# Createroner/InSAR-Unet-CA

Hardware: AMD Instinct MI355X
Metric: InSAR tiles/sec (fwd+bwd) U-Net-CA 256x256 (higher is better)
Workload: dtype bf16; 1 GPU; U-Net-CA (in=2, classes=2, use_se) bf16, batch 16x2x256x256 per GPU, Dice+CE + Adam(lr=1e-4) training on synthetic InSAR tiles; global_batch=16, parallelism=dp1

## Files before the change

insar_unet_ca_amd/csrc/wgrad.hip:

```cpp
#include "common.h"

typedef __attribute__((ext_vector_type(8))) short bf16x8_t;
typedef __attribute__((ext_vector_type(4))) short s16x4_t;
typedef __attribute__((ext_vector_type(4))) float f32x4_t;

#define WG_BKP 64

struct WgradArgs {
  const char* x; const char* dy; const int32_t* tabx; const int32_t* tabdy; float* part;
  long long ksteps;
  int nsplit, ntaps, steps_per_split;
  int Cx, cx_off, Cin; int Cdy, cdy_off, Cout;
  int mtc, ntc;
  int offx[12], offdy[12];
  long long tabx_tap_stride;
};


template <int RB>
__device__ __forceinline__ int wg_swz(int row) {
  if constexpr (RB == 256) return (row & 7) << 1;
  else return ((row >> 1) & 3) << 1;
}

template <typename T, int TM, int TN, int NW>
struct WgradCfg {
  static constexpr int ES = sizeof(T);
  static constexpr int THREADS = NW * 64;
  static constexpr int SUBX = (TM * ES > 256) ? TM * ES / 256 : 1, SUBY = (TN * ES > 256) ? TN * ES / 256 : 1;
  static constexpr int RBX = TM * ES / SUBX, RBY = TN * ES / SUBY;
  static constexpr int X_STAGE = WG_BKP * TM * ES, Y_STAGE = WG_BKP * TN * ES;
  static constexpr int STAGE = X_STAGE + Y_STAGE;
  static constexpr int LDS_BYTES = 2 * STAGE + 128;
  static constexpr int CPRX = RBX / 16, CPRY = RBY / 16;
  static constexpr int NX = X_STAGE / 16 / THREADS;
  static constexpr int NY = Y_STAGE / 16 / THREADS;
  static constexpr int MTW = TM / 32, NTW = TN / (NW / 2) / 16;
};

template <typename T, int TM, int TN, int NW>
__global__ __launch_bounds__(NW * 64, (NW == 4 ? 2 : 1)) void wgrad_kernel(WgradArgs a) {
  using Cfg = WgradCfg<T, TM, TN, NW>;
  constexpr int WG_THREADS = Cfg::THREADS;
  constexpr int ES = Cfg::ES;
  constexpr int MTW = Cfg::MTW, NTW = Cfg::NTW;
  extern __shared__ __attribute__((aligned(16))) char smem[];
  int* soff = (int*)(smem + 2 * Cfg::STAGE);

  const int tid = threadIdx.x, lane = tid & 63, wave = tid >> 6;
  int t;
  {
    const int nwg = gridDim.x, bid = blockIdx.x;
    const int q = nwg >> 3, r = nwg & 7, xcd = bid & 7;
    t = (xcd < r ? xcd * (q + 1) : r * (q + 1) + (xcd - r) * q) + (bid >> 3);
  }
  const int tap = t % a.ntaps; t /= a.ntaps;
  const int ni = t % a.ntc; t /= a.ntc;
  const int mi = t % a.mtc; t /= a.mtc;
  const int split = t;

  if (tid == WG_THREADS - 1) {
#pragma unroll
    for (int i = 0; i < 12; ++i) { soff[i] = a.offx[i]; soff[12 + i] = a.offdy[i]; }
  }
  __syncthreads();
  const long long offx = soff[tap], offdy = soff[12 + tap];

  const long long ks0 = (long long)split * a.steps_per_split;
  long long ks1 = ks0 + a.steps_per_split;
  if (ks1 > a.ksteps) ks1 = a.ksteps;

  const long long xcol = ((long long)a.cx_off + mi * TM) * ES;
  const long long ycol = ((long long)a.cdy_off + ni * TN) * ES;
  int xrow_i[Cfg::NX], yrow_i[Cfg::NY];
  int xoff_i[Cfg::NX], yoff_i[Cfg::NY];
#pragma unroll
  for (int i = 0; i < Cfg::NX; ++i) {
    const int q = i * WG_THREADS + tid;
    const int sub = q / (WG_BKP * Cfg::CPRX), row = (q / Cfg::CPRX) % WG_BKP, pos = q % Cfg::CPRX;
    xrow_i[i] = row;
    xoff_i[i] = sub * Cfg::RBX + (pos ^ wg_swz<Cfg::RBX>(row)) * 16;
  }
#pragma unroll
  for (int i = 0; i < Cfg::NY; ++i) {
    const int q = i * WG_THREADS + tid;
    const int sub = q / (WG_BKP * Cfg::CPRY), row = (q / Cfg::CPRY) % WG_BKP, pos = q % Cfg::CPRY;
    yrow_i[i] = row;
    yoff_i[i] = sub * Cfg::RBY + (pos ^ wg_swz<Cfg::RBY>(row)) * 16;
  }
  const char* xbase = a.x + offx * a.Cx * ES + xcol;
  const char* ybase = a.dy + offdy * a.Cdy * ES + ycol;
  const long long xpitch = (long long)a.Cx * ES, ypitch = (long long)a.Cdy * ES;

  int32_t px[Cfg::NX], py[Cfg::NY];
  const int32_t* tabx_tap = a.tabx + (long long)tap * a.tabx_tap_stride;
  auto load_tabs = [&](long long ks) {
#pragma unroll
    for (int i = 0; i < Cfg::NX; ++i) px[i] = tabx_tap[ks * WG_BKP + xrow_i[i]];
#pragma unroll
    for (int i = 0; i < Cfg::NY; ++i) py[i] = a.tabdy[ks * WG_BKP + yrow_i[i]];
  };
  const uint32_t lds0 = lds_offset_of(smem);
  auto stage = [&](int buf) {
    const uint32_t lx = lds0 + buf * Cfg::STAGE + wave * 1024;
#pragma unroll
    for (int i = 0; i < Cfg::NX; ++i)
      lds_dma16_untracked(xbase + (long long)px[i] * xpitch + xoff_i[i], lx + i * (WG_THREADS * 16));
    const uint32_t ly = lx + Cfg::X_STAGE;
#pragma unroll
    for (int i = 0; i < Cfg::NY; ++i)
      lds_dma16_untracked(ybase + (long long)py[i] * ypitch + yoff_i[i], ly + i * (WG_THREADS * 16));
  };

  f32x4_t acc[MTW][NTW];
#pragma unroll
  for (int i = 0; i < MTW; ++i)
#pragma unroll
    for (int j = 0; j < NTW; ++j) acc[i][j] = (f32x4_t){0.f, 0.f, 0.f, 0.f};

  const int wm = wave & 1, wn = wave >> 1;
  const int r16 = lane & 15, kq = lane >> 4;

  if (ks0 < ks1) {
    load_tabs(ks0);
    stage(0);
    if (ks0 + 1 < ks1) load_tabs(ks0 + 1);
    dma_drain_and_barrier();
    for (long long ks = ks0; ks < ks1; ++ks) {
      const int buf = (int)((ks - ks0) & 1);
      if (ks + 1 < ks1) {
        stage(buf ^ 1);
        if (ks + 2 < ks1) load_tabs(ks + 2);
      }
      const char* sX = smem + buf * Cfg::STAGE;
      const char* sY = sX + Cfg::X_STAGE;
      if constexpr (ES == 2) {
#pragma unroll
        for (int s = 0; s < 2; ++s) {
          bf16x8_t xf[MTW], yf[NTW];
#pragma unroll
          for (int h = 0; h < 2; ++h) {
            const int sel = h ^ (kq & 1);
            const int row = s * 32 + kq * 8 + sel * 4 + (r16 >> 2);
#pragma unroll
            for (int mt = 0; mt < MTW; ++mt) {
              const int colw = (wm * (TM / 2) + mt * 16 + (r16 & 3) * 4) * 2;
              int sub = 0, colb = colw;
              if constexpr (Cfg::SUBX > 1) { sub = colw / Cfg::RBX; colb = colw % Cfg::RBX; }
              const int pc = (colb >> 4) ^ wg_swz<Cfg::RBX>(row);
              const char* p = sX + sub * (WG_BKP * Cfg::RBX) + row * Cfg::RBX + pc * 16 + (colb & 15);
              s16x4_t v = __builtin_amdgcn_ds_read_tr16_b64_v4i16((__attribute__((address_space(3))) s16x4_t*)p);
              xf[mt][4 * h + 0] = v[0]; xf[mt][4 * h + 1] = v[1]; xf[mt][4 * h + 2] = v[2]; xf[mt][4 * h + 3] = v[3];
            }
#pragma unroll
            for (int nt = 0; nt < NTW; ++nt) {
              const int colw = (wn * (NTW * 16) + nt * 16 + (r16 & 3) * 4) * 2;
              int sub = 0, colb = colw;
              if constexpr (Cfg::SUBY > 1) { sub = colw / Cfg::RBY; colb = colw % Cfg::RBY; }
              const int pc = (colb >> 4) ^ wg_swz<Cfg::RBY>(row);
              const char* p = sY + sub * (WG_BKP * Cfg::RBY) + row * Cfg::RBY + pc * 16 + (colb & 15);
              s16x4_t v = __builtin_amdgcn_ds_read_tr16_b64_v4i16((__attribute__((address_space(3))) s16x4_t*)p);
              yf[nt][4 * h + 0] = v[0]; yf[nt][4 * h + 1] = v[1]; yf[nt][4 * h + 2] = v[2]; yf[nt][4 * h + 3] = v[3];
            }
          }
#pragma unroll
          for (int mt = 0; mt < MTW; ++mt)
#pragma unroll
            for (int nt = 0; nt < NTW; ++nt)
              acc[mt][nt] = __builtin_amdgcn_mfma_f32_16x16x32_bf16(xf[mt], yf[nt], acc[mt][nt], 0, 0, 0);
        }
      } else {
#pragma unroll 4
        for (int jj = 0; jj < WG_BKP / 4; ++jj) {
          const int row = jj * 4 + kq;
          float xf[MTW], yf[NTW];
#pragma unroll
          for (int mt = 0; mt < MTW; ++mt) {
            const int colw = (wm * (TM / 2) + mt * 16 + r16) * 4;
            const int sub = colw / Cfg::RBX, colb = colw % Cfg::RBX;
            const int pc = (colb >> 4) ^ wg_swz<Cfg::RBX>(row);
            xf[mt] = *(const float*)(sX + sub * (WG_BKP * Cfg::RBX) + row * Cfg::RBX + pc * 16 + (colb & 15));
          }
#pragma unroll
          for (int nt = 0; nt < NTW; ++nt) {
            const int colw = (wn * (NTW * 16) + nt * 16 + r16) * 4;
            const int sub = colw / Cfg::RBY, colb = colw % Cfg::RBY;
            const int pc = (colb >> 4) ^ wg_swz<Cfg::RBY>(row);
            yf[nt] = *(const float*)(sY + sub * (WG_BKP * Cfg::RBY) + row * Cfg::RBY + pc * 16 + (colb & 15));
          }
#pragma unroll
          for (int mt = 0; mt < MTW; ++mt)
#pragma unroll
            for (int nt = 0; nt < NTW; ++nt)
              acc[mt][nt] = __builtin_amdgcn_mfma_f32_16x16x4f32(xf[mt], yf[nt], acc[mt][nt], 0, 0, 0);
        }
      }
      dma_drain_and_barrier();
    }
  }

  float* out = a.part + ((long long)split * a.ntaps + tap) * a.Cout * a.Cin;
#pragma unroll
  for (int mt = 0; mt < MTW; ++mt)
#pragma unroll
    for (int nt = 0; nt < NTW; ++nt) {
      const int ci = mi * TM + wm * (TM / 2) + mt * 16 + kq * 4;
      const int co = ni * TN + wn * (NTW * 16) + nt * 16 + r16;
      *(f32x4_t*)(out + (long long)co * a.Cin + ci) = acc[mt][nt];
    }
}

template <typename T, int TM, int TN, int NW>
static int launch_wgrad(WgradArgs& a, hipStream_t s) {
  using Cfg = WgradCfg<T, TM, TN, NW>;
  static std::atomic<uint64_t> attr_mask{0};
  {
    hipError_t e = insar_set_lds_once(attr_mask, (const void*)wgrad_kernel<T, TM, TN, NW>, Cfg::LDS_BYTES);
    if (e != hipSuccess) INSAR_FAIL(-(int)e, "insar_wgrad: hipFuncSetAttribute: %s", hipGetErrorString(e));
  }
  a.mtc = a.Cin / TM; a.ntc = a.Cout / TN;
  const long long grid = (long long)a.nsplit * a.ntaps * a.mtc * a.ntc;
  if (grid > 0x7fffffffLL) INSAR_FAIL(INSAR_E_SHAPE, "insar_wgrad: grid too large");
  hipLaunchKernelGGL((wgrad_kernel<T, TM, TN, NW>), dim3((unsigned)grid), dim3(Cfg::THREADS), Cfg::LDS_BYTES, s, a);
  INSAR_CHECK_LAUNCH("insar_wgrad");
  return INSAR_OK;
}

extern "C" int insar_wgrad_tile(int32_t C, int32_t dtype) {
  if (dtype != INSAR_BF16) return (C % 128) == 0 ? 128 : 64;
  const int cap = insar_knob(KNOB_WGRAD_TILE_MAX);
  if (cap > 0 && cap < 256) return (C % 128) == 0 ? 128 : 64;
  return (C % 256) == 0 ? 256 : ((C % 128) == 0 ? 128 : 64);
}

static void wgrad_tile_pair(int Cin, int Cout, int dtype, int& tm, int& tn) {
  tm = insar_wgrad_tile(Cin, dtype); tn = insar_wgrad_tile(Cout, dtype);
  if (dtype != INSAR_BF16) { if (!(tm == 128 && tn == 128)) tm = tn = 64; return; }
  if (tm == 256 && tn == 256) return;
  tm = tm > 128 ? 128 : tm; tn = tn > 128 ? 128 : tn;
}
extern "C" int insar_wgrad_tile_pair(int32_t Cin, int32_t Cout, int32_t dtype) {
  int tm, tn;
  wgrad_tile_pair(Cin, Cout, dtype, tm, tn);
  return (tm << 16) | tn;
}

extern "C" int insar_wgrad(const InsarWgrad* d, void* stream) {
  if (!d || !d->x.ptr || !d->dy.ptr || !d->tabx || !d->tabdy || !d->part) INSAR_FAIL(INSAR_E_ARG, "insar_wgrad: null pointer");
  int rc;
  if ((rc = insar_check_act(&d->x, "insar_wgrad", "x"))) return rc;
  if ((rc = insar_check_act(&d->dy, "insar_wgrad", "dy"))) return rc;
  if (d->x.dtype != d->dy.dtype) INSAR_FAIL(INSAR_E_DTYPE, "insar_wgrad: x/dy dtype differ");
  if (d->Mpad < WG_BKP || d->Mpad % WG_BKP) INSAR_FAIL(INSAR_E_SHAPE, "insar_wgrad: Mpad must be a positive multiple of 64");
  if (d->nsplit < 1 || d->ntaps < 1 || d->ntaps > 12) INSAR_FAIL(INSAR_E_SHAPE, "insar_wgrad: nsplit/ntaps");
  const int Cin = d->x.c_len, Cout = d->dy.c_len;
  if (Cin % 64 || Cout % 64) INSAR_FAIL(INSAR_E_SHAPE, "insar_wgrad: Cin=%d/Cout=%d must be multiples of 64", Cin, Cout);
  WgradArgs a;
  a.x = (const char*)d->x.ptr; a.dy = (const char*)d->dy.ptr; a.tabx = d->tabx; a.tabdy = d->tabdy; a.part = d->part;
  a.ksteps = d->Mpad / WG_BKP;
  a.nsplit = d->nsplit; a.ntaps = d->ntaps;
  a.steps_per_split = (int)((a.ksteps + d->nsplit - 1) / d->nsplit);
  a.Cx = d->x.C; a.cx_off = d->x.c_off; a.Cin = Cin;
  a.Cdy = d->dy.C; a.cdy_off = d->dy.c_off; a.Cout = Cout;
  for (int t = 0; t < 12; ++t) { a.offx[t] = t < d->ntaps ? d->offx[t] : 0; a.offdy[t] = t < d->ntaps ? d->offdy[t] : 0; }
  a.tabx_tap_stride = d->tabx_tap_stride;
  hipStream_t s = (hipStream_t)stream;
  int tm, tn;
  wgrad_tile_pair(Cin, Cout, d->x.dtype, tm, tn);
  if (d->x.dtype == INSAR_BF16) {
    if (tm == 256 && tn == 256) return launch_wgrad<bf16_t, 256, 256, 8>(a, s);
    if (tm == 128 && tn == 128) return launch_wgrad<bf16_t, 128, 128, 4>(a, s);
    if (tm == 128) return launch_wgrad<bf16_t, 128, 64, 4>(a, s);
    if (tn == 128) return launch_wgrad<bf16_t, 64, 128, 4>(a, s);
    return launch_wgrad<bf16_t, 64, 64, 4>(a, s);
  }
  if (tm == 128 && tn == 128) return launch_wgrad<float, 128, 128, 8>(a, s);
  return launch_wgrad<float, 64, 64, 4>(a, s);
}

__global__ void wgrad_fold_kernel(const float4* __restrict__ in, float4* __restrict__ out, long long slab4, int nsplit,
                                  int group) {
  const int g = blockIdx.y;
  const int s0 = g * group;
  int s1 = s0 + group; if (s1 > nsplit) s1 = nsplit;
  for (long long e = blockIdx.x * (long long)blockDim.x + threadIdx.x; e < slab4; e += (long long)gridDim.x * blockDim.x) {
    float4 acc = make_float4(0.f, 0.f, 0.f, 0.f);
#pragma unroll 8
    for (int sp = s0; sp < s1; ++sp) {
      const float4 v = in[(long long)sp * slab4 + e];
      acc.x += v.x; acc.y += v.y; acc.z += v.z; acc.w += v.w;
    }
    out[(long long)g * slab4 + e] = acc;
  }
}

extern "C" int insar_wgrad_fold(const float* part_in, float* part_out, int64_t slab_floats, int32_t nsplit, int32_t group,
                                void* stream) {
  if (!part_in || !part_out) INSAR_FAIL(INSAR_E_ARG, "insar_wgrad_fold: null pointer");
  if (slab_floats < 4 || (slab_floats & 3) || nsplit < 1 || group < 1) INSAR_FAIL(INSAR_E_SHAPE, "insar_wgrad_fold: bad shape");
  const long long slab4 = slab_floats / 4;
  const int groups = (nsplit + group - 1) / group;
  dim3 grid(insar_grid_cap((slab4 + 255) / 256, 1024), groups);
  hipLaunchKernelGGL(wgrad_fold_kernel, grid, dim3(256), 0, (hipStream_t)stream, (const float4*)part_in, (float4*)part_out,
                     slab4, nsplit, group);
  INSAR_CHECK_LAUNCH("insar_wgrad_fold");
  return INSAR_OK;
}

#define WR_CIT 128
template <bool VEC>
__global__ void wgrad_reduce_kernel(const float* __restrict__ part, float* __restrict__ grad, int nsplit, int ntaps,
                                    int Co, int Ci, int layout, int accumulate) {
  __shared__ float t[WR_CIT * 12];
  const int co = blockIdx.x, ci0 = blockIdx.y * WR_CIT;
  const int nci = (Ci - ci0) < WR_CIT ? (Ci - ci0) : WR_CIT;
  const long long total = (long long)Co * Ci;
  const long long slab = total * ntaps;
  if constexpr (VEC) {
    const int nc4 = nci >> 2;
    for (int idx = threadIdx.x; idx < ntaps * nc4; idx += blockDim.x) {
      const int tap = idx / nc4, c = (idx - tap * nc4) << 2;
      const float* p = part + (long long)tap * total + (long long)co * Ci + ci0 + c;
      float4 s = make_float4(0.f, 0.f, 0.f, 0.f);
      int sp = 0;
      for (; sp + 8 <= nsplit; sp += 8) {
        float4 v[8];
#pragma unroll
        for (int u = 0; u < 8; ++u) v[u] = *(const float4*)(p + (long long)(sp + u) * slab);
#pragma unroll
        for (int u = 0; u < 4; ++u) { v[u].x += v[u + 4].x; v[u].y += v[u + 4].y; v[u].z += v[u + 4].z; v[u].w += v[u + 4].w; }
        s.x += (v[0].x + v[1].x) + (v[2].x + v[3].x); s.y += (v[0].y + v[1].y) + (v[2].y + v[3].y);
        s.z += (v[0].z + v[1].z) + (v[2].z + v[3].z); s.w += (v[0].w + v[1].w) + (v[2].w + v[3].w);
      }
      for (; sp < nsplit; ++sp) {
        const float4 v = *(const float4*)(p + (long long)sp * slab);
        s.x += v.x; s.y += v.y; s.z += v.z; s.w += v.w;
      }
      t[(c + 0) * ntaps + tap] = s.x; t[(c + 1) * ntaps + tap] = s.y;
      t[(c + 2) * ntaps + tap] = s.z; t[(c + 3) * ntaps + tap] = s.w;
    }
  } else {
  for (int idx = threadIdx.x; idx < ntaps * nci; idx += blockDim.x) {
    const int tap = idx / nci, c = idx - tap * nci;
    const float* p = part + (long long)tap * total + (long long)co * Ci + ci0 + c;
    float s0 = 0.f, s1 = 0.f, s2 = 0.f, s3 = 0.f;
    int sp = 0;
    for (; sp + 4 <= nsplit; sp += 4) {
      s0 += p[(long long)sp * slab]; s1 += p[(long long)(sp + 1) * slab];
      s2 += p[(long long)(sp + 2) * slab]; s3 += p[(long long)(sp + 3) * slab];
    }
    for (; sp < nsplit; ++sp) s0 += p[(long long)sp * slab];
    t[c * ntaps + tap] = (s0 + s1) + (s2 + s3);
  }
  }
  __syncthreads();
  if (layout == 0) {
    float* g = grad + ((long long)co * Ci + ci0) * ntaps;
    for (int j = threadIdx.x; j < nci * ntaps; j += blockDim.x) g[j] = accumulate ? g[j] + t[j] : t[j];
  } else {
    for (int j = threadIdx.x; j < nci * ntaps; j += blockDim.x) {
      const int c = j / ntaps, tap = j - c * ntaps;
      float* g = grad + ((long long)(ci0 + c) * Co + co) * ntaps + tap;
      *g = accumulate ? *g + t[j] : t[j];
    }
  }
}

extern "C" int insar_wgrad_reduce(const float* part, float* grad, int32_t nsplit, int32_t ntaps, int32_t Co, int32_t Ci,
                                  int32_t layout, int32_t accumulate, void* stream) {
  if (!part || !grad) INSAR_FAIL(INSAR_E_ARG, "insar_wgrad_reduce: null pointer");
  if (layout != 0 && layout != 1) INSAR_FAIL(INSAR_E_ARG, "insar_wgrad_reduce: layout");
  if (ntaps < 1 || ntaps > 12 || Co < 1 || Ci < 1 || nsplit < 1) INSAR_FAIL(INSAR_E_SHAPE, "insar_wgrad_reduce: bad shape");
  dim3 grid(Co, (Ci + WR_CIT - 1) / WR_CIT);
  if ((Ci & 3) == 0 && insar_aligned16(part))
    hipLaunchKernelGGL(wgrad_reduce_kernel<true>, grid, dim3(256), 0, (hipStream_t)stream, part, grad, nsplit, ntaps, Co, Ci,
                       layout, accumulate);
  else
    hipLaunchKernelGGL(wgrad_reduce_kernel<false>, grid, dim3(256), 0, (hipStream_t)stream, part, grad, nsplit, ntaps, Co, Ci,
                       layout, accumulate);
  INSAR_CHECK_LAUNCH("insar_wgrad_reduce");
  return INSAR_OK;
}
```

insar_unet_ca_amd/engine.py:

```python
from __future__ import annotations

import contextlib
import ctypes as C
import os
from typing import Dict, List, Optional

import torch

from . import _lib, tape
from ._lib import InsarAct, InsarBnFinalize, InsarBnSeBwd, InsarIgemm, InsarSa, InsarSeFwd, InsarWgrad, call, ptr
from .tape import tape_py

BN_ROW_PIX = 128
WG_BKP = 64


def _round_up(a: int, b: int) -> int:
    return (a + b - 1) // b * b


class Act:

    def __init__(self, buf: torch.Tensor, B: int, H: int, W: int, Ctot: int, c_off: int, c_len: int):
        self.buf, self.B, self.H, self.W, self.C, self.c_off, self.c_len = buf, B, H, W, Ctot, c_off, c_len
        self.code = _lib.dtype_code(buf.dtype)
        self.desc = InsarAct(buf.data_ptr(), B, H, W, Ctot, c_off, c_len, self.code, 0)
        self.ref = C.byref(self.desc)

    @staticmethod
    def alloc(B, H, W, Cn, dtype, device) -> "Act":
        nbytes = B * (H + 2) * (W + 2) * Cn * (2 if dtype == torch.bfloat16 else 4)
        if nbytes >= 2 ** 32:
            raise _lib.InsarError(f"activation buffer of {nbytes} bytes exceeds the 4 GiB addressing budget")
        return Act(torch.zeros((B, H + 2, W + 2, Cn), dtype=dtype, device=device), B, H, W, Cn, 0, Cn)

    def slice(self, c_off: int, c_len: int) -> "Act":
        return Act(self.buf, self.B, self.H, self.W, self.C, self.c_off + c_off, c_len)

    def nchw(self) -> torch.Tensor:
        v = self.buf[:, 1:-1, 1:-1, self.c_off:self.c_off + self.c_len]
        return v.permute(0, 3, 1, 2).float().contiguous()


class Ctx:

    def __init__(self, device: torch.device, dtype: torch.dtype):
        self.device, self.dtype = device, dtype
        self.code = _lib.dtype_code(dtype)
        self.esize = 2 if dtype == torch.bfloat16 else 4
        self.ch = 16 // self.esize
        self._colsum_tmp: Dict[int, torch.Tensor] = {}
        self.side = (torch.cuda.Stream(device=device, priority=int(os.environ.get("INSAR_SIDE_PRIORITY", "0")))
                     if device.type == "cuda" and os.environ.get("INSAR_SIDE_STREAM", "1") != "0" else None)
        mask = os.environ.get("INSAR_SIDE_CU_MASK")
        if self.side is not None and mask:
            self.side = _cu_masked_stream(device, mask)
        self._side_busy = False
        self._wgrad_part: Optional[torch.Tensor] = None
        self._wgrad_fold: Optional[torch.Tensor] = None
        self._tables: Dict[tuple, torch.Tensor] = {}
        self._consts: Dict[tuple, torch.Tensor] = {}

    def f32(self, *shape) -> torch.Tensor:
        return torch.zeros(shape, dtype=torch.float32, device=self.device)

    def const(self, value: float, n: int) -> torch.Tensor:
        key = (value, n)
        if key not in self._consts:
            self._consts[key] = torch.full((n,), value, dtype=torch.float32, device=self.device)
        return self._consts[key]

    @contextlib.contextmanager
    def side_stream(self):
        if self.side is None or (PROFILER is not None and PROFILER.alone):
            yield
            return
        prev = self._side_enter()
        try:
            yield
        finally:
            self._side_exit(prev)

    def _side_enter(self):
        if tape.REC is not None:
            tape.REC.op("side_enter")
        prev = torch.cuda.current_stream()
        self.side.wait_stream(prev)
        torch.cuda.set_stream(self.side)
        return prev

    def _side_exit(self, prev) -> None:
        torch.cuda.set_stream(prev)
        self._side_busy = True
        if tape.REC is not None:
            tape.REC.op("side_exit")

    def join_side(self) -> None:
        if tape.REC is not None:
            tape.REC.op("join")
        if self._side_busy:
            torch.cuda.current_stream().wait_stream(self.side)
            self._side_busy = False

    def colsum(self, part: torch.Tensor, out: torch.Tensor, segments: int, rows: int, cols: int,
               accumulate: bool = False, ld: Optional[int] = None, part_off: int = 0) -> None:
        s = _lib.stream_ptr()
        tmp = self._colsum_tmp.get(s)
        need = ((rows + 127) // 128) * segments * cols if rows > 256 else 0
        if tmp is None or need > tmp.numel():
            tmp = self._colsum_tmp[s] = torch.empty(max(need, 1 << 20), dtype=torch.float32, device=self.device)
        if ld is None:
            call("insar_colsum", ptr(part), ptr(out), segments, rows, cols, int(accumulate), ptr(tmp), tmp.numel(), s)
        else:
            call("insar_colsum_ld", ptr(part) + 4 * part_off, ptr(out), segments, rows, cols, ld, int(accumulate), ptr(tmp), tmp.numel(), s)

    def colsum_into_grads(self, part: torch.Tensor, rows: int, views: List[torch.Tensor]) -> None:
        total = sum(v.numel() for v in views)
        adjacent = all(views[i + 1].data_ptr() == views[i].data_ptr() + 4 * views[i].numel() for i in range(len(views) - 1))
        if adjacent:
            self.colsum(part, views[0], 1, rows, total)
            return
        off = 0
        for v in views:
            self.colsum(part, v, 1, rows, v.numel(), ld=total, part_off=off)
            off += v.numel()

    def wgrad_part(self, floats: int) -> torch.Tensor:
        if self._wgrad_part is None or self._wgrad_part.numel() < floats:
            self._wgrad_part = torch.empty(floats, dtype=torch.float32, device=self.device)
        return self._wgrad_part

    def wgrad_finish(self, part: torch.Tensor, grad: torch.Tensor, nsplit: int, ntaps: int, cout: int, cin: int,
                     layout: int) -> None:
        s = _lib.stream_ptr()
        slab = ntaps * cout * cin
        if nsplit > 48:
            group = 8 if nsplit <= 96 else 16
            groups = (nsplit + group - 1) // group
            if self._wgrad_fold is None or self._wgrad_fold.numel() < groups * slab:
                self._wgrad_fold = torch.empty(groups * slab, dtype=torch.float32, device=self.device)
            call("insar_wgrad_fold", ptr(part), ptr(self._wgrad_fold), slab, nsplit, group, s)
            part, nsplit = self._wgrad_fold, groups
        call("insar_wgrad_reduce", ptr(part), ptr(grad), nsplit, ntaps, cout, cin, layout, 0, s)

    def pixel_table(self, B, H, W, s, Hb, Wb, tail) -> torch.Tensor:
        key = (B, H, W, s, Hb, Wb, tail)
        if key not in self._tables:
            mpad = _round_up(B * H * W, WG_BKP)
            t = torch.empty(mpad, dtype=torch.int32, device=self.device)
            call("insar_pixel_table", ptr(t), mpad, B, H, W, s, Hb, Wb, tail, _lib.stream_ptr())
            self._tables[key] = t
        return self._tables[key]


def _cu_masked_stream(device: torch.device, spec: str):
    n, _, stride = spec.partition(":")
    n, stride = int(n), int(stride or 1)
    words = [0] * 8
    for i in range(n):
        b = (i * stride) % 256 + (i * stride) // 256
        words[b // 32] |= 1 << (b % 32)
    hip = C.CDLL("libamdhip64.so")
    stream = C.c_void_p()
    arr = (C.c_uint32 * 8)(*words)
    with torch.cuda.device(device):
        rc = hip.hipExtStreamCreateWithCUMask(C.byref(stream), 8, arr)
    if rc != 0:
        raise _lib.InsarError(f"hipExtStreamCreateWithCUMask failed ({rc})")
    return torch.cuda.ExternalStream(stream.value, device=device)


def _taps_table(self, B: int, Ho: int, Wo: int, s: int, Hb: int, Wb: int, taps) -> torch.Tensor:
    key = ("taps", B, Ho, Wo, s, Hb, Wb, tuple(taps))
    if key not in self._tables:
        mpad = _round_up(B * Ho * Wo, WG_BKP)
        t = torch.empty(len(taps) * mpad, dtype=torch.int32, device=self.device)
        dy = (C.c_int8 * 12)(*([a for a, _ in taps] + [0] * (12 - len(taps))))
        dx = (C.c_int8 * 12)(*([b for _, b in taps] + [0] * (12 - len(taps))))
        call("insar_pixel_table_taps", ptr(t), mpad, B, Ho, Wo, s, Hb, Wb, len(taps), C.addressof(dy), C.addressof(dx),
             _lib.stream_ptr())
        self._tables[key] = t
    return self._tables[key]


Ctx.taps_table = _taps_table


class GemmWeight:

    def __init__(self, ctx: Ctx, param: torch.nn.Parameter, kind: str):
        self.ctx, self.param, self.kind = ctx, param, kind
        if kind == "conv3":
            co, ci = param.shape[0], param.shape[1]
            T = param.shape[2] * param.shape[3]
            self._spec = {"fwd": (T, co, ci, 1, ci * T, T), "dgrad": (T, ci, co, 1, T, ci * T)}
        else:
            ci, co = param.shape[0], param.shape[1]
            self._spec = {"fwd": (4, co, ci, 1, 4, co * 4), "dgrad": (4, ci, co, 1, co * 4, 4)}
        self._buf = {k: torch.empty(v[:3], dtype=ctx.dtype, device=ctx.device) for k, v in self._spec.items()}
        self._key = {"fwd": None, "dgrad": None}

    def key(self):
        return (self.param._version, self.param.data_ptr())

    def master(self) -> torch.Tensor:
        w = self.param.detach()
        if w.dtype != torch.float32 or not w.is_contiguous():
            raise _lib.InsarError("weights must be contiguous float32 parameters")
        return w

    def _get(self, which: str) -> torch.Tensor:
        if self._key[which] != self.key():
            if tape.REC is not None:
                tape.REC.bad("weight re-layout inside a recording")
            T, N, K, st, sn, sk = self._spec[which]
            call("insar_weight_prep", ptr(self.master()), ptr(self._buf[which]), self.ctx.code, T, N, K, st, sn, sk,
                 _lib.stream_ptr())
            self._key[which] = self.key()
        return self._buf[which]

    def fwd(self) -> torch.Tensor:
        return self._get("fwd")

    def dgrad(self) -> torch.Tensor:
        return self._get("dgrad")


class WeightSet:

    def __init__(self, ctx: Ctx, weights: List[GemmWeight]):
        self.ctx, self.weights = ctx, weights
        self._jobs = None
        self._ptrs = None
        self._total = 0
        self._by_stage = None

    def stage_sets(self, groups) -> List["WeightSet"]:
        if self._by_stage is None:
            owner = {id(p): i for i, g in enumerate(groups) for p in g}
            buckets = [[] for _ in groups]
            for w in self.weights:
                buckets[owner[id(w.param)]].append(w)
            self._by_stage = [WeightSet(self.ctx, b) if b else None for b in buckets]
        return self._by_stage

    def stale(self) -> bool:
        return any(w._key["fwd"] != w.key() or w._key["dgrad"] != w.key() for w in self.weights)

    def refresh(self) -> None:
        tape.tape_live(self._refresh_now)

    def _refresh_now(self) -> None:
        if not self.stale():
            return
        ptrs = tuple(w.param.data_ptr() for w in self.weights)
        if self._jobs is None or ptrs != self._ptrs:
            rows, tile0 = [], 0
            for w in self.weights:
                a, b = w.param.shape[0], w.param.shape[1]
                T = w.param.shape[2] * w.param.shape[3]
                oab, oba = (w._buf["fwd"], w._buf["dgrad"]) if w.kind == "conv3" else (w._buf["dgrad"], w._buf["fwd"])
                rows.append([w.master().data_ptr(), oab.data_ptr(), oba.data_ptr(), a, b, T, tile0, w.ctx.code])
                tile0 += ((a + 31) // 32) * ((b + 31) // 32)
            self._jobs = torch.tensor(rows, dtype=torch.int64).to(self.ctx.device)
            self._ptrs, self._total = ptrs, tile0
        call("insar_weight_prep_pair_batch", ptr(self._jobs), self._jobs.shape[0], self._total, _lib.stream_ptr())
        for w in self.weights:
            w._key["fwd"] = w._key["dgrad"] = w.key()


class KernelTimer:

    def __init__(self, alone: bool = True):
        self.alone = alone
        self.elapsed = 0.0
        self.records: Dict[str, list] = {}

    def run(self, tag: str, flops: float, fn, nbytes: float = 0.0) -> None:
        e0, e1 = torch.cuda.Event(enable_timing=True), torch.cuda.Event(enable_timing=True)
        e0.record()
        fn()
        e1.record()
        self.records.setdefault(tag, []).append((e0, e1, flops, nbytes))

    def summary(self) -> Dict[str, dict]:
        torch.cuda.synchronize()
        out = {}
        for tag, recs in self.records.items():
            ms = sum(r[0].elapsed_time(r[1]) for r in recs)
            fl = sum(r[2] for r in recs)
            out[tag] = {"launches": len(recs), "ms": ms, "flops": fl, "bytes": sum(r[3] for r in recs),
                        "avg_us": 1e3 * ms / max(len(recs), 1), "tflops": fl / (ms * 1e-3) / 1e12 if ms > 0 else 0.0}
        return out


PROFILER: Optional[KernelTimer] = None
SPLIT_COEF = os.environ.get("INSAR_SPLIT_COEF", "0") == "1"
POOL_FUSE = os.environ.get("INSAR_POOL_FUSE", "1") != "0"
SMALL_WGRAD_FUSE = os.environ.get("INSAR_SMALL_WGRAD_FUSE", "1") != "0"
SMALL_WGRAD_MAIN = os.environ.get("INSAR_SMALL_WGRAD_MAIN", "1") != "0"
PREP_SIDE = os.environ.get("INSAR_PREP_SIDE", "1") != "0"
OUTC_FUSE = os.environ.get("INSAR_OUTC_FUSE", "1") != "0"
WGRAD_GRID_CAP = int(os.environ.get("INSAR_WGRAD_GRID_CAP", "200"))
COEF_FUSE = os.environ.get("INSAR_COEF_FUSE", "1") != "0"
COEF_SIMPLE = os.environ.get("INSAR_COEF_SIMPLE", "1") != "0"
OUTC_WGRAD_FUSE = os.environ.get("INSAR_OUTC_WGRAD_FUSE", "1") != "0"
WGRAD_FILL_T = float(os.environ.get("INSAR_WGRAD_FILL_T", "0.7"))
WGRAD_FILL_DL = float(os.environ.get("INSAR_WGRAD_FILL_DL", "0.5"))
WGRAD_FILL_ALONE = float(os.environ.get("INSAR_WGRAD_FILL_ALONE", "1.0"))
WGRAD_FILL_SMALL = float(os.environ.get("INSAR_WGRAD_FILL_SMALL", os.environ.get("INSAR_WGRAD_FILL", "0.5")))
WGRAD_FILL = float(os.environ.get("INSAR_WGRAD_FILL", "0.5"))
WGRAD_ROWS = os.environ.get("INSAR_WGRAD_ROWS", "1") != "0"
WGRAD_K = os.environ.get("INSAR_WGRAD_K", "0") != "0"
WGRAD_K_TILES = set(os.environ.get("INSAR_WGRAD_K_TILES", "128x64,128x128").split(","))
WGRAD_X = os.environ.get("INSAR_WGRAD_X", "1") != "0"
WGRAD_Y = int(os.environ.get("INSAR_WGRAD_Y", "0"))
FLAT_PP = int(os.environ.get("INSAR_FLAT_PP", "1"))
FLAT_PERSIST = int(os.environ.get("INSAR_FLAT_PERSIST", "2"))
IGEMM_PP = int(os.environ.get("INSAR_IGEMM_PP", "1"))
STAT_PREFOLD_ROWS = int(os.environ.get("INSAR_STAT_PREFOLD_ROWS", "1024"))
FLAT_ROWS = os.environ.get("INSAR_FLAT_ROWS", "1") != "0"
FLAT2 = int(os.environ.get("INSAR_FLAT2", "1"))
FLAT2_PERSIST = int(os.environ.get("INSAR_FLAT2_PERSIST", "1"))
FLAT2_KMAX = int(os.environ.get("INSAR_FLAT2_KMAX", "512"))
BSTAT_FUSE = os.environ.get("INSAR_BSTAT_FUSE", "1") != "0"
BSTAT_C64 = os.environ.get("INSAR_BSTAT_C64", "1") != "0"
WGRAD_LATE = os.environ.get("INSAR_WGRAD_ORDER", "before") == "after"


_TAPS3 = [(r - 1, s - 1) for r in range(3) for s in range(3)]
_TAPS3_DGRAD = [(1 - r, 1 - s) for r in range(3) for s in range(3)]
_TAPS2 = [(a, b) for a in range(2) for b in range(2)]


def _launch(tag, flops, fn, nbytes=0.0) -> None:
    if PROFILER is None:
        fn()
        return
    tag, flops, nbytes = (v() if callable(v) else v for v in (tag, flops, nbytes))
    PROFILER.run(tag, flops, fn, nbytes)


def _igemm(x: Act, y: Act, w, N: int, Ho: int, Wo: int, stride: int, taps, mode: int,
           bias: Optional[torch.Tensor] = None, stats: Optional[torch.Tensor] = None, oob: bool = False,
           add: Optional[Act] = None, out_stride: int = 1, out_off=(0, 0), bstat=None, gate: Optional[Act] = None) -> None:
    d = InsarIgemm()
    if bstat is not None:
        d.bstat.y, d.bstat.scale, d.bstat.shift = bstat[0].buf.data_ptr(), ptr(bstat[1]), ptr(bstat[2])
    d.x, d.y = x.desc, y.desc
    d.w, d.bias, d.stats = (w if isinstance(w, int) else ptr(w)), ptr(bias), ptr(stats)
    d.N, d.Ho, d.Wo, d.stride, d.ntaps, d.mode = N, Ho, Wo, stride, len(taps), mode
    d.flags = (_lib.IGEMM_OOB_ZERO if oob else 0) | (_lib.IGEMM_PINGPONG if IGEMM_PP else 0)
    d.out_stride, d.out_oy, d.out_ox = out_stride, out_off[0], out_off[1]
    if add is not None:
        if add.C != y.C or add.c_off != y.c_off or add.buf.dtype != y.buf.dtype or add.buf.shape != y.buf.shape:
            raise _lib.InsarError("igemm: `add` must have the output's buffer layout")
        d.add = add.buf.data_ptr()
    if gate is not None:
        if gate.C != y.C or gate.c_off != y.c_off or gate.buf.dtype != y.buf.dtype or gate.buf.shape != y.buf.shape:
            raise _lib.InsarError("igemm: `gate` must have the output's buffer layout")
        d.gate = gate.buf.data_ptr()
    for i, (dy, dx) in enumerate(taps):
        d.dy[i], d.dx[i] = dy, dx
    if PROFILER is not None:
        flops = 2.0 * x.B * Ho * Wo * N * x.c_len * len(taps)
        bm = call("insar_igemm_tile_rows", x.B * Ho * Wo, N)
        bn = call("insar_igemm_tile_cols_dt", x.B * Ho * Wo, N, x.code)
        if oob and x.code == _lib.F32:
            bn = 64
        tag = "igemm_kernel<%s, %d, %d, %d%s>%s" % ("float" if x.code == _lib.F32 else "bf16_t", bm, bn,
                                                    3 if bm == 256 and bn < 256 else 2, ", oob" if oob else "",
                                                    " +bstat" if bstat is not None else "")
        es = 2 if x.code == _lib.BF16 else 4
        nbytes = es * (x.B * x.H * x.W * x.c_len + y.B * y.H * y.W * y.c_len + len(taps) * N * x.c_len)
        PROFILER.run(tag, flops, lambda: call("insar_igemm", C.byref(d), _lib.stream_ptr()), nbytes)
        return
    call("insar_igemm", C.byref(d), _lib.stream_ptr())


def _flat_persist(flip: int) -> bool:
    return FLAT_PERSIST == 2 or (FLAT_PERSIST == 1 and not (flip & 1))


def _flat_flags(flip: int, x: Act) -> int:
    two = FLAT2 and x.code == _lib.BF16
    rows = two and FLAT2 == 1 and call("insar_conv3x3_flat2_rows_ok", x.ref, 64)
    persist = _flat2_persist(flip) if two else _flat_persist(flip)
    return (32 if two else 0) | (8 if rows else 0) | (4 if (persist and not (two and FLAT2 == 2)) else 0)


def _flat2_persist(flip: int) -> bool:
    return FLAT2_PERSIST == 2 or (FLAT2_PERSIST == 1 and not (flip & 1))


def _rows_flags(x: Act, N: int, K: Optional[int] = None, flip: int = 0) -> int:
    if not FLAT_ROWS or x.code != _lib.BF16 or not call("insar_conv3x3_flat_rows_ok", x.ref, N):
        return 0
    M = x.B * x.H * x.W
    two = (FLAT2 == 1 and (N % 128) == 0 and (M // 256) * (N // 128) >= 2 * torch.cuda.get_device_properties(x.buf.device).multi_processor_count
           and call("insar_conv3x3_flat2_rows_ok", x.ref, N))
    if call("insar_igemm_tile_cols_dt", M, N, x.code) == 256:
        return (8 | 32 | (4 if _flat2_persist(flip) else 0)) if (two and (x.c_len if K is None else K) <= FLAT2_KMAX) else 0
    narrow = (N % 128) != 0 or (M // 256) * (N // 128) < 256
    if two:
        return 8 | 32 | (4 if _flat2_persist(flip) else 0)
    return 8 | (16 if narrow else 0)


def _conv3x3_flat(x: Act, y: Act, w: torch.Tensor, flip: int, stats: Optional[torch.Tensor], bstat=None, geo: int = 0) -> None:
    flags = flip | (2 if (FLAT_PP or geo) else 0) | (0 if geo else _flat_flags(flip, x)) | geo
    if bstat is not None:
        bs = _lib.InsarBstat(bstat[0].buf.data_ptr(), ptr(bstat[1]), ptr(bstat[2]))
        fn = lambda: call("insar_conv3x3_flat_bstat", x.ref, y.ref, ptr(w), flags, ptr(stats), C.byref(bs), _lib.stream_ptr())
    else:
        fn = lambda: call("insar_conv3x3_flat", x.ref, y.ref, ptr(w), flags, ptr(stats), _lib.stream_ptr())
    def tag():
        if flags & 32:
            return "conv3x3_flat2_kernel<%d, %s, %d>" % (128 if y.c_len % 128 == 0 else 64, "true" if bstat is not None else "false", (flags >> 3) & 1)
        return "conv3x3_flat_kernel<%s, %d>%s%s" % ("float" if x.code == _lib.F32 else "bf16_t",
                                                    128 if (y.c_len % 128 == 0 and not (geo & 16)) else 64,
                                                    (" row tiles" + (" dilated" if (geo >> 8) & 15 else "")) if geo else "", " +bstat" if bstat is not None else "")

    def nbytes():
        es = 2 if x.code == _lib.BF16 else 4
        return float(x.B * x.H * x.W * (x.c_len + y.c_len * (2 if bstat is not None else 1)) * es + 9 * x.c_len * y.c_len * es)
    _launch(tag, lambda: 2.0 * x.B * x.H * x.W * y.c_len * x.c_len * 9, fn, nbytes)


def _conv3x3_c64(x: Act, y: Act, w: torch.Tensor, flip: int, stats: Optional[torch.Tensor], bstat=None) -> None:
    if bstat is not None:
        bs = _lib.InsarBstat(bstat[0].buf.data_ptr(), ptr(bstat[1]), ptr(bstat[2]))
        fn = lambda: call("insar_conv3x3_c64_bstat", x.ref, y.ref, ptr(w), flip, ptr(stats), C.byref(bs), _lib.stream_ptr())
    else:
        fn = lambda: call("insar_conv3x3_c64", x.ref, y.ref, ptr(w), flip, ptr(stats), _lib.stream_ptr())
    _launch(lambda: "conv3x3_c64_kernel<2>" + (" +bstat" if bstat is not None else ""), lambda: 2.0 * x.B * x.H * x.W * 64 * 64 * 9, fn)


def _wgrad_tiles(cin: int, cout: int, code: int):
    pair = call("insar_wgrad_tile_pair", cin, cout, code)
    return pair >> 16, pair & 0xffff


def _launch_wgrad(d: InsarWgrad, M: int, cin: int, cout: int, ntaps: int, code: int) -> None:
    def tag():
        tm, tn = _wgrad_tiles(cin, cout, code)
        return "wgrad_kernel<%s, %d, %d, %d>" % ("float" if code == _lib.F32 else "bf16_t", tm, tn,
# ... 972 lines not shown
```

Before: 2346 tiles/s.

## Fuse split-K fold into wgrad reduce with multi-column tiles and padded LDS

Removes the separate wgrad fold kernel and its intermediate buffer. The reduce kernel now sums split-K partials directly, grouping them so the summation order matches the old fold, and each block handles several output columns with one item per thread. LDS staging gains padding to avoid bank conflicts, and a smaller-block path is used when the grid would be small. The aim is to save a launch and the extra memory round trip of the folded slabs. The cost is more template variants and fixed LDS capacity limits that can now reject a shape.

```diff
diff --git a/insar_unet_ca_amd/csrc/wgrad.hip b/insar_unet_ca_amd/csrc/wgrad.hip
--- a/insar_unet_ca_amd/csrc/wgrad.hip
+++ b/insar_unet_ca_amd/csrc/wgrad.hip
@@ -1,4 +1,5 @@
 #include "common.h"
+#include <type_traits>
 
 typedef __attribute__((ext_vector_type(8))) short bf16x8_t;
 typedef __attribute__((ext_vector_type(4))) short s16x4_t;
@@ -307,62 +308,157 @@
   return INSAR_OK;
 }
 
-#define WR_CIT 128
-template <bool VEC>
-__global__ void wgrad_reduce_kernel(const float* __restrict__ part, float* __restrict__ grad, int nsplit, int ntaps,
-                                    int Co, int Ci, int layout, int accumulate) {
-  __shared__ float t[WR_CIT * 12];
-  const int co = blockIdx.x, ci0 = blockIdx.y * WR_CIT;
-  const int nci = (Ci - ci0) < WR_CIT ? (Ci - ci0) : WR_CIT;
+#define WR_LDS_FLOATS 3328
+
+__device__ __forceinline__ void wr_load(float4& v, const float* p) { v = *(const float4*)p; }
+__device__ __forceinline__ void wr_load(float& v, const float* p) { v = *p; }
+__device__ __forceinline__ float4 wr_add(float4 a, float4 b) { return make_float4(a.x + b.x, a.y + b.y, a.z + b.z, a.w + b.w); }
+__device__ __forceinline__ float wr_add(float a, float b) { return a + b; }
+__device__ __forceinline__ void wr_zero(float4& v) { v = make_float4(0.f, 0.f, 0.f, 0.f); }
+__device__ __forceinline__ void wr_zero(float& v) { v = 0.f; }
+template <typename V>
+__device__ __forceinline__ V wr_tree8(const V (&v)[8]) {
+  return wr_add(wr_add(wr_add(v[0], v[4]), wr_add(v[1], v[5])), wr_add(wr_add(v[2], v[6]), wr_add(v[3], v[7])));
+}
+
+template <bool FULL, int KC, typename V>
+__device__ __forceinline__ void wr_group_partials(const float* p, long long slab, int nsplit, int group, int gi, int klen,
+                                                  V (&g)[8]) {
+#pragma unroll
+  for (int u = 0; u < 8; ++u) wr_zero(g[u]);
+  for (int k = 0; k < klen; k += KC) {
+    V v[8][KC];
+#pragma unroll
+    for (int u = 0; u < 8; ++u)
+#pragma unroll
+      for (int kk = 0; kk < KC; ++kk) {
+        int sl = (gi + u) * group + k + kk;
+        if (!FULL && sl > nsplit - 1) sl = nsplit - 1;
+        wr_load(v[u][kk], p + (long long)sl * slab);
+      }
+#pragma unroll
+    for (int kk = 0; kk < KC; ++kk)
+#pragma unroll
+      for (int u = 0; u < 8; ++u)
+        if (FULL || (gi + u) * group + k + kk < nsplit) g[u] = wr_add(g[u], v[u][kk]);
+  }
+}
+
+template <int NT, bool VEC, int KC>
+__global__ __launch_bounds__(NT) void wgrad_reduce_kernel(const float* __restrict__ part, float* __restrict__ grad, int nsplit,
+                                                          int group, int ntaps, int Co, int Ci, int layout, int accumulate,
+                                                          int cot, int cit, int pitch) {
+  typedef typename std::conditional<VEC, float4, float>::type V;
+  constexpr int W = VEC ? 4 : 1;
+  __shared__ float t[WR_LDS_FLOATS];
+  const int co0 = blockIdx.x * cot, ci0 = blockIdx.y * cit;
+  const int ncol = (Co - co0) < cot ? (Co - co0) : cot;
+  const int nci = (Ci - ci0) < cit ? (Ci - ci0) : cit;
+  const int ncu = nci / W;
+  const int nitems = ntaps * ncol * ncu;
   const long long total = (long long)Co * Ci;
   const long long slab = total * ntaps;
-  if constexpr (VEC) {
-    const int nc4 = nci >> 2;
-    for (int idx = threadIdx.x; idx < ntaps * nc4; idx += blockDim.x) {
-      const int tap = idx / nc4, c = (idx - tap * nc4) << 2;
-      const float* p = part + (long long)tap * total + (long long)co * Ci + ci0 + c;
-      float4 s = make_float4(0.f, 0.f, 0.f, 0.f);
-      int sp = 0;
-      for (; sp + 8 <= nsplit; sp += 8) {
-        float4 v[8];
-#pragma unroll
-        for (int u = 0; u < 8; ++u) v[u] = *(const float4*)(p + (long long)(sp + u) * slab);
-#pragma unroll
-        for (int u = 0; u < 4; ++u) { v[u].x += v[u + 4].x; v[u].y += v[u + 4].y; v[u].z += v[u + 4].z; v[u].w += v[u + 4].w; }
-        s.x += (v[0].x + v[1].x) + (v[2].x + v[3].x); s.y += (v[0].y + v[1].y) + (v[2].y + v[3].y);
-        s.z += (v[0].z + v[1].z) + (v[2].z + v[3].z); s.w += (v[0].w + v[1].w) + (v[2].w + v[3].w);
-      }
-      for (; sp < nsplit; ++sp) {
-        const float4 v = *(const float4*)(p + (long long)sp * slab);
-        s.x += v.x; s.y += v.y; s.z += v.z; s.w += v.w;
-      }
-      t[(c + 0) * ntaps + tap] = s.x; t[(c + 1) * ntaps + tap] = s.y;
-      t[(c + 2) * ntaps + tap] = s.z; t[(c + 3) * ntaps + tap] = s.w;
+  const bool ok = (int)threadIdx.x < nitems;
+  const int id = ok ? threadIdx.x : 0;
+  const int tap = (int)((id + 0.5f) * __frcp_rn((float)(ncol * ncu))), r = id - tap * (ncol * ncu);
+  const int col = (int)((r + 0.5f) * __frcp_rn((float)ncu)), c = (r - col * ncu) * W;
+  const float* p = part + (long long)tap * total + (long long)(co0 + col) * Ci + ci0 + c;
+  V s;
+  wr_zero(s);
+  if constexpr (KC == 0) {
+    int sp = 0;
+    for (; sp + 8 <= nsplit; sp += 8) {
+      V v[8];
+#pragma unroll
+      for (int u = 0; u < 8; ++u) wr_load(v[u], p + (long long)(sp + u) * slab);
+      s = wr_add(s, wr_tree8(v));
+    }
+    if (sp < nsplit) {
+      const int n = nsplit - sp;
+      V v[8];
+#pragma unroll
+      for (int u = 0; u < 8; ++u) wr_load(v[u], p + (long long)(sp + (u < n ? u : n - 1)) * slab);
+#pragma unroll
+      for (int u = 0; u < 8; ++u)
+        if (u < n) s = wr_add(s, v[u]);
     }
   } else {
-  for (int idx = threadIdx.x; idx < ntaps * nci; idx += blockDim.x) {
-    const int tap = idx / nci, c = idx - tap * nci;
-    const float* p = part + (long long)tap * total + (long long)co * Ci + ci0 + c;
-    float s0 = 0.f, s1 = 0.f, s2 = 0.f, s3 = 0.f;
-    int sp = 0;
-    for (; sp + 4 <= nsplit; sp += 4) {
-      s0 += p[(long long)sp * slab]; s1 += p[(long long)(sp + 1) * slab];
-      s2 += p[(long long)(sp + 2) * slab]; s3 += p[(long long)(sp + 3) * slab];
-    }
-    for (; sp < nsplit; ++sp) s0 += p[(long long)sp * slab];
-    t[c * ntaps + tap] = (s0 + s1) + (s2 + s3);
-  }
+    const int ng = (nsplit + group - 1) / group;
+    V g[8];
+    int gi = 0;
+    for (; (gi + 8) * group <= nsplit; gi += 8) {
+      wr_group_partials<true, KC>(p, slab, nsplit, group, gi, group, g);
+      s = wr_add(s, wr_tree8(g));
+    }
+    if (gi < ng) {
+      const int nr = ng - gi;
+      const int left = nsplit - gi * group;
+      wr_group_partials<false, KC>(p, slab, nsplit, group, gi, left < group ? left : group, g);
+      if (nr == 8) s = wr_add(s, wr_tree8(g));
+      else {
+#pragma unroll
+        for (int u = 0; u < 7; ++u)
+          if (u < nr) s = wr_add(s, g[u]);
+      }
+    }
+  }
+  const int row = nci * ntaps, run = ncol * ntaps;
+  if (ok) {
+    if (layout == 0) {
+      int l = col * row + c * ntaps + tap;
+      if constexpr (VEC) {
+        t[l + (l >> 5)] = s.x; l += ntaps; t[l + (l >> 5)] = s.y; l += ntaps; t[l + (l >> 5)] = s.z; l += ntaps; t[l + (l >> 5)] = s.w;
+      } else {
+        t[l + (l >> 5)] = s;
+      }
+    } else {
+      const int e = col * ntaps + tap, a = c * pitch + e + (e >> 2);
+      if constexpr (VEC) {
+        t[a] = s.x; t[a + pitch] = s.y; t[a + 2 * pitch] = s.z; t[a + 3 * pitch] = s.w;
+      } else {
+        t[a] = s;
+      }
+    }
   }
   __syncthreads();
   if (layout == 0) {
-    float* g = grad + ((long long)co * Ci + ci0) * ntaps;
-    for (int j = threadIdx.x; j < nci * ntaps; j += blockDim.x) g[j] = accumulate ? g[j] + t[j] : t[j];
+    for (int cl = 0; cl < ncol; ++cl) {
+      float* g = grad + ((long long)(co0 + cl) * Ci + ci0) * ntaps;
+      for (int e = threadIdx.x; e < row; e += NT) {
+        const int l = cl * row + e;
+        const float v = t[l + (l >> 5)];
+        g[e] = accumulate ? g[e] + v : v;
+      }
+    }
   } else {
-    for (int j = threadIdx.x; j < nci * ntaps; j += blockDim.x) {
-      const int c = j / ntaps, tap = j - c * ntaps;
-      float* g = grad + ((long long)(ci0 + c) * Co + co) * ntaps + tap;
-      *g = accumulate ? *g + t[j] : t[j];
-    }
+    const int qs = NT / run, rs = NT - qs * run;
+    int ci = (int)((threadIdx.x + 0.5f) * __frcp_rn((float)run)), e = threadIdx.x - ci * run;
+    float* g = grad + ((long long)ci0 * Co + co0) * ntaps;
+    while (ci < nci) {
+      const float v = t[ci * pitch + e + (e >> 2)];
+      float* o = g + (long long)ci * Co * ntaps + e;
+      *o = accumulate ? *o + v : v;
+      ci += qs; e += rs;
+      if (e >= run) { e -= run; ++ci; }
+    }
+  }
+}
+
+template <int NT, bool VEC, int KC>
+static void wr_launch2(dim3 grid, hipStream_t s, const float* part, float* grad, int nsplit, int group, int ntaps, int Co, int Ci,
+                       int layout, int accumulate, int cot, int cit, int pitch) {
+  hipLaunchKernelGGL((wgrad_reduce_kernel<NT, VEC, KC>), grid, dim3(NT), 0, s, part, grad, nsplit, group, ntaps, Co, Ci, layout,
+                     accumulate, cot, cit, pitch);
+}
+template <int NT, int KC>
+static void wr_launch(bool vec, dim3 grid, hipStream_t s, const float* part, float* grad, int nsplit, int group, int ntaps,
+                      int Co, int Ci, int layout, int accumulate, int cot, int cit, int pitch) {
+  if (group == 1) {
+    if (vec) wr_launch2<NT, true, 0>(grid, s, part, grad, nsplit, group, ntaps, Co, Ci, layout, accumulate, cot, cit, pitch);
+    else wr_launch2<NT, false, 0>(grid, s, part, grad, nsplit, group, ntaps, Co, Ci, layout, accumulate, cot, cit, pitch);
+  } else {
+    if (vec) wr_launch2<NT, true, KC>(grid, s, part, grad, nsplit, group, ntaps, Co, Ci, layout, accumulate, cot, cit, pitch);
+    else wr_launch2<NT, false, KC>(grid, s, part, grad, nsplit, group, ntaps, Co, Ci, layout, accumulate, cot, cit, pitch);
   }
 }
 
@@ -371,13 +467,32 @@
   if (!part || !grad) INSAR_FAIL(INSAR_E_ARG, "insar_wgrad_reduce: null pointer");
   if (layout != 0 && layout != 1) INSAR_FAIL(INSAR_E_ARG, "insar_wgrad_reduce: layout");
   if (ntaps < 1 || ntaps > 12 || Co < 1 || Ci < 1 || nsplit < 1) INSAR_FAIL(INSAR_E_SHAPE, "insar_wgrad_reduce: bad shape");
-  dim3 grid(Co, (Ci + WR_CIT - 1) / WR_CIT);
-  if ((Ci & 3) == 0 && insar_aligned16(part))
-    hipLaunchKernelGGL(wgrad_reduce_kernel<true>, grid, dim3(256), 0, (hipStream_t)stream, part, grad, nsplit, ntaps, Co, Ci,
-                       layout, accumulate);
-  else
-    hipLaunchKernelGGL(wgrad_reduce_kernel<false>, grid, dim3(256), 0, (hipStream_t)stream, part, grad, nsplit, ntaps, Co, Ci,
-                       layout, accumulate);
+  const int group = nsplit <= 48 ? 1 : nsplit <= 96 ? 8 : 16;
+  const bool vec = (Ci & 3) == 0 && insar_aligned16(part);
+  const int w = vec ? 4 : 1;
+  const bool three = ntaps % 3 == 0;
+  int nt = three ? 576 : 512;
+  int cit = (vec && layout == 0) ? 128 : 32;
+  int cw = Ci < cit ? Ci : cit;
+  int cot = nt / (ntaps * (cw / w));
+  cot = cot < 1 ? 1 : cot > Co ? Co : cot;
+  if (vec && (long long)((Co + cot - 1) / cot) * ((Ci + cit - 1) / cit) < 256) {
+    nt = three ? 192 : 128;
+    cit = 32;
+    cw = Ci < cit ? Ci : cit;
+    cot = nt / (ntaps * (cw / w));
+    cot = cot < 1 ? 1 : cot > Co ? Co : cot;
+  }
+  const int tile = cot * cw * ntaps, run = cot * ntaps;
+  const int pitch = (run + run / 4 + 1) | 1;
+  const int lds = layout == 0 ? tile + tile / 32 + 1 : cw * pitch;
+  if (ntaps * cot * (cw / w) > nt || lds > WR_LDS_FLOATS) INSAR_FAIL(INSAR_E_SHAPE, "insar_wgrad_reduce: tile does not fit");
+  dim3 grid((Co + cot - 1) / cot, (Ci + cit - 1) / cit);
+  hipStream_t s = (hipStream_t)stream;
+  if (nt == 576) wr_launch<576, 2>(vec, grid, s, part, grad, nsplit, group, ntaps, Co, Ci, layout, accumulate, cot, cit, pitch);
+  else if (nt == 512) wr_launch<512, 2>(vec, grid, s, part, grad, nsplit, group, ntaps, Co, Ci, layout, accumulate, cot, cit, pitch);
+  else if (nt == 192) wr_launch<192, 4>(vec, grid, s, part, grad, nsplit, group, ntaps, Co, Ci, layout, accumulate, cot, cit, pitch);
+  else wr_launch<128, 4>(vec, grid, s, part, grad, nsplit, group, ntaps, Co, Ci, layout, accumulate, cot, cit, pitch);
   INSAR_CHECK_LAUNCH("insar_wgrad_reduce");
   return INSAR_OK;
 }
diff --git a/insar_unet_ca_amd/engine.py b/insar_unet_ca_amd/engine.py
--- a/insar_unet_ca_amd/engine.py
+++ b/insar_unet_ca_amd/engine.py
@@ -132,16 +132,7 @@
 
     def wgrad_finish(self, part: torch.Tensor, grad: torch.Tensor, nsplit: int, ntaps: int, cout: int, cin: int,
                      layout: int) -> None:
-        s = _lib.stream_ptr()
-        slab = ntaps * cout * cin
-        if nsplit > 48:
-            group = 8 if nsplit <= 96 else 16
-            groups = (nsplit + group - 1) // group
-            if self._wgrad_fold is None or self._wgrad_fold.numel() < groups * slab:
-                self._wgrad_fold = torch.empty(groups * slab, dtype=torch.float32, device=self.device)
-            call("insar_wgrad_fold", ptr(part), ptr(self._wgrad_fold), slab, nsplit, group, s)
-            part, nsplit = self._wgrad_fold, groups
-        call("insar_wgrad_reduce", ptr(part), ptr(grad), nsplit, ntaps, cout, cin, layout, 0, s)
+        call("insar_wgrad_reduce", ptr(part), ptr(grad), nsplit, ntaps, cout, cin, layout, 0, _lib.stream_ptr())
 
     def pixel_table(self, B, H, W, s, Hb, Wb, tail) -> torch.Tensor:
         key = (B, H, W, s, Hb, Wb, tail)
```

Measured after the change: 2349 tiles/s (median of 2 runs). Within noise of the previous version (+0.1%).
